# DoumanAsh/compu

Measured on AMD Instinct MI355X. Metric: decompressed GB/s (whole node), batched 64 KiB DEFLATE blocks; % HBM peak, higher is better.
Workload: dtype u8

## Files before the change

### compu_amd/csrc/inflate_unit.h

```cpp
#pragma once
#include "chip_internal.h"
#include "wave_checksums.h"

namespace chip {

typedef uint32_t u32x2 __attribute__((ext_vector_type(2)));
typedef uint32_t u32x4 __attribute__((ext_vector_type(4)));
typedef u32x4 u32x4_u __attribute__((aligned(1)));
typedef u32x4 u32x4_a4 __attribute__((aligned(4)));
template <typename T>
__device__ __forceinline__ GAS T *rdfirst_gptr(T *p)
{
    return (GAS T *)rdfirst_ptr(p);
}

#ifndef CHIP_PHASE_FN
#define CHIP_PHASE_FN __attribute__((always_inline))
#endif

#ifndef CHIP_INFLATE_SPEC
#define CHIP_INFLATE_SPEC 0
#endif
#ifndef CHIP_INFLATE_MARKERS
#define CHIP_INFLATE_MARKERS 0
// ... 471 lines not shown
    if (allow_gzip && b0 == 0x1f && b1 == 0x8b) {
        wrap = 2;
        if (avail < 4) return CHIP_NEED_INPUT;
        const uint32_t flg = gin[3];
        if (gin[2] != 8) return Z_DATA_ERROR;
        if (flg & 0xe0) return Z_DATA_ERROR;
        if (avail < 10) return CHIP_NEED_INPUT;
        uint32_t k = 10;
        if (flg & 4) {
            if (avail < k + 2) return CHIP_NEED_INPUT;
            uint32_t xlen = gin[k] | ((uint32_t)gin[k + 1] << 8);
            k += 2;
            if (avail - k < xlen) return CHIP_NEED_INPUT;
            k += xlen;
        }
        for (uint32_t bit = 8; bit <= 16; bit <<= 1) {
            if (!(flg & bit)) continue;
            for (;;) {
                uint32_t idx = k + lane_id();
                uint64_t z = __ballot(idx < avail && gin[idx] == 0);
                if (z) {
                    k += (uint32_t)__ffsll((long long)z);
                    break;
                }
                if (avail - k <= 64) return CHIP_NEED_INPUT;
                k += 64;
            }
        }
        if (flg & 2) {
            if (avail < k + 2) return CHIP_NEED_INPUT;
            uint32_t crc = wave_crc32(tab, gin, k);
            if ((crc & 0xffffu) != (gin[k] | ((uint32_t)gin[k + 1] << 8))) return Z_DATA_ERROR;
            k += 2;
        }
        hdr = k;
        return ST_RUNNING;
    }
    if (!allow_zlib) return Z_DATA_ERROR;
    if (((b0 << 8) | b1) % 31u) return Z_DATA_ERROR;
    if ((b0 & 15u) != 8) return Z_DATA_ERROR;
    if ((b0 >> 4) + 8 > 15) return Z_DATA_ERROR;
    wrap = 1;
    hdr = 2;
    if (b1 & 0x20) {
        if (avail < 6) return CHIP_NEED_INPUT;
        hdr = 6;
        return CHIP_NEED_DICT;
    }
    return ST_RUNNING;
}

struct __attribute__((packed)) U32u { uint32_t v; };
struct __attribute__((packed)) U16u { uint16_t v; };
struct __attribute__((packed)) U128u { uint32_t x, y, z, w; };
typedef LDS_AS uint8_t lds_u8;

__device__ void wave_copy_stored(uint8_t *gdst, const uint32_t *g32, uint32_t total_dw, uint32_t so, uint32_t n)
{
    const uint32_t lane = lane_id();
    const uint8_t *gsrc = (const uint8_t *)g32 + so;
    uint32_t head = (uint32_t)((16u - ((uintptr_t)gdst & 15u)) & 15u);
    if (head > n) head = n;
    if (lane < head) gdst[lane] = gsrc[lane];
    uint32_t done = head;
    const uint32_t body = (n - done) & ~15u;
    if (body) {
        uint4 *d16 = (uint4 *)(gdst + done);
        const U128u *s16 = (const U128u *)(gsrc + done);
        const uint32_t cnt = body >> 4;
        uint32_t i = lane;
#ifdef CHIP_STORED_NT_LD
#define CHIP_STORED_LD(p) __builtin_nontemporal_load(p)
#else
#define CHIP_STORED_LD(p) (*(p))
#endif
#ifndef CHIP_STORED_PLAIN_ST
#define CHIP_STORED_ST(v, p) __builtin_nontemporal_store(v, p)
#else
#define CHIP_STORED_ST(v, p) (*(p) = (v))
#endif
#ifndef CHIP_STORED_DEPTH
#define CHIP_STORED_DEPTH 2
#endif
        for (; i + 64u * (CHIP_STORED_DEPTH - 1) < cnt; i += 64u * CHIP_STORED_DEPTH) {
            u32x4 v[CHIP_STORED_DEPTH];
#pragma unroll
            for (int k = 0; k < CHIP_STORED_DEPTH; k++) v[k] = CHIP_STORED_LD((const u32x4_u *)(s16 + i + 64u * k));
#pragma unroll
            for (int k = 0; k < CHIP_STORED_DEPTH; k++) CHIP_STORED_ST(v[k], (u32x4 *)(d16 + i + 64u * k));
        }
        for (; i < cnt; i += 64u) {
            const U128u a = s16[i];
            d16[i] = make_uint4(a.x, a.y, a.z, a.w);
        }
        done += body;
    }
    const uint32_t tail = n - done;
    if (lane < tail) gdst[done + lane] = gsrc[done + lane];
    (void)total_dw;
}

__device__ __forceinline__ uint32_t small_mod(uint32_t off, uint32_t d)
{
    uint32_t q = (uint32_t)(((float)off + 0.5f) * __builtin_amdgcn_rcpf((float)d));
    return off - q * d;
}
struct ChunkLds {
    uint32_t *out;
    uint2 *mq;
    uint32_t *tok;
    lds_u8 *trash;
};

__device__ __forceinline__ ChunkLds chunk_lds(WaveLds &L)
{
    ChunkLds c;
    c.out = L.fl.out;
    c.mq = L.fl.mq;
    c.tok = L.fl.tok;
    c.trash = (lds_u8 *)L.fl.trash;
    return c;
}

__device__ __forceinline__ void lds_put(lds_u8 *d, lds_u8 *trash, const U128u &v, uint32_t n)
{
    ((LDS_AS U32u *)(n >= 4 ? d : trash))->v = v.x;
    ((LDS_AS U32u *)((n >= 8 ? d : trash) + 4))->v = v.y;
    ((LDS_AS U32u *)((n >= 12 ? d : trash) + 8))->v = v.z;
    ((LDS_AS U32u *)((n >= 16 ? d : trash) + 12))->v = v.w;
    const uint32_t w = n < 4 ? v.x : n < 8 ? v.y : n < 12 ? v.z : v.w;
    lds_u8 *const t = d + (n & 12u);
    const bool two = (n & 2u) != 0, one = (n & 1u) != 0;
    ((LDS_AS U16u *)(two ? t : trash))->v = (uint16_t)w;
    *(one ? (two ? t + 2 : t) : trash) = (uint8_t)(two ? w >> 16 : w);
}

__device__ __forceinline__ void copy_one_match(lds_u8 *img, const uint8_t *base, uint32_t mis, uint32_t x, uint32_t len, uint32_t dist)
{
    const uint32_t lane = lane_id();
    const int32_t sx = (int32_t)x - (int32_t)dist;
    for (uint32_t i = lane; i < len; i += 64) {
        const int32_t s = sx + (int32_t)(dist >= len ? i : small_mod(i, dist));
        uint8_t b = 0;
        if (s < (int32_t)mis) b = ((GAS const uint8_t *)base)[s];
        if (s >= (int32_t)mis) b = img[s];
        img[x + i] = b;
    }
    LSYNC();
}

struct Round {
    uint32_t x, len, dist;
    bool glob;
    U128u v0, v1;
};

__device__ __forceinline__ void round_issue(Round &r, const ChunkLds &C, const uint8_t *base, uint32_t mis, uint32_t qh, uint32_t nr,
                                            bool glob_ok)
{
    const uint32_t lane = lane_id();
    const bool act = lane < nr;
    const uint32_t qi = (qh + lane) & (MQ_CAP - 1u);
    const uint2 e = C.mq[qi];
    r.x = e.x;
    const uint32_t ld = act ? e.y : 0u;
    r.len = ld & 0xffffu;
    r.dist = ld >> 16;
    const int32_t sx = (int32_t)r.x - (int32_t)r.dist;
    r.glob = glob_ok && r.len != 0 && r.len <= COPY_LANE_MAX && sx + (int32_t)r.len <= (int32_t)mis;
    r.v0 = U128u{0, 0, 0, 0};
    r.v1 = U128u{0, 0, 0, 0};
#ifndef CHIP_EXP_NO_GLOB
    if (r.glob) {
        const u32x4_u t = *(GAS const u32x4_u *)(base + sx);
        r.v0 = U128u{t.x, t.y, t.z, t.w};
    }
#endif
#ifndef CHIP_EXP_NO_GLOB
    if (r.glob && r.len > 16u) {
        const u32x4_u t = *(GAS const u32x4_u *)(base + sx + 16);
        r.v1 = U128u{t.x, t.y, t.z, t.w};
    }
#endif
}

__device__ __forceinline__ void round_finish(const Round &r, const ChunkLds &C, const uint8_t *base, uint32_t mis STAT_PARAM)
{
    const uint32_t lane = lane_id();
    lds_u8 *const img = (lds_u8 *)C.out;
    const int32_t sx = (int32_t)r.x - (int32_t)r.dist;
    uint64_t pend = __ballot(r.len != 0);
    STAT_ADD(14, 1);
    while (pend) {
        const uint32_t f = (uint32_t)__ffsll((long long)pend) - 1u;
        const uint32_t wp = rdlane(r.x, f);
        const bool mine = (pend >> lane) & 1ull;
        const bool loc = sx >= (int32_t)mis && (uint32_t)sx + r.len <= wp;
        const bool ready = mine && r.len <= COPY_LANE_MAX && (r.glob || loc);
        const uint64_t rm = __ballot(ready);
        if (!((rm >> f) & 1ull)) {
            STAT_ADD(15, 1);
            copy_one_match(img, base, mis, wp, rdlane(r.len, f), rdlane(r.dist, f));
            pend &= pend - 1ull;
            continue;
        }
        STAT_ADD(12, 1);
        uint32_t rem = ready ? r.len : 0u;
#pragma unroll
        for (uint32_t it = 0; it < COPY_LANE_MAX / 16; it++) {
            if (it && !__any(rem != 0)) break;
            U128u v = it ? r.v1 : r.v0;
            if (rem && !r.glob) {
                const lds_u8 *sp = img + sx + (int32_t)(16u * it);
                v.x = ((const LDS_AS U32u *)sp)->v;
                v.y = ((const LDS_AS U32u *)(sp + 4))->v;
                v.z = ((const LDS_AS U32u *)(sp + 8))->v;
                v.w = ((const LDS_AS U32u *)(sp + 12))->v;
            }
            const uint32_t n = rem < 16u ? rem : 16u;
            lds_put(img + r.x + 16u * it, C.trash, v, n);
            rem -= n;
        }
        LSYNC();
        pend &= ~rm;
    }
}

__device__ __forceinline__ uint32_t lane_gather(uint32_t x, uint32_t src)
{
    return (uint32_t)__builtin_amdgcn_ds_bpermute((int)(src << 2), (int)x);
}

__device__ uint32_t token_end(const WaveLds &L, const InWin &w, uint32_t p, bool second)
{
    const uint32_t i = p >> 5;
    const uint32_t d0 = i < w.total_dw ? w.g32[i] : 0u, d1 = i + 1u < w.total_dw ? w.g32[i + 1u] : 0u, d2 = i + 2u < w.total_dw ? w.g32[i + 2u] : 0u;
    const uint32_t lo = __builtin_amdgcn_alignbit(d1, d0, p), hi = __builtin_amdgcn_alignbit(d2, d1, p);
    const uint32_t r = L.lit_root[lo & ((1u << LIT_ROOT) - 1u)];
    const uint32_t e = pool_at(L, r, lo);
    const uint32_t n1 = __builtin_amdgcn_ubfe(e, 10, 5);
    const uint32_t w2 = __builtin_amdgcn_alignbit(hi, lo, n1);
    if (!(e & F_LEN)) {
        if (!second) return p + n1;
        const uint32_t r2 = L.lit_root[w2 & ((1u << LIT_ROOT) - 1u)];
        return p + n1 + __builtin_amdgcn_ubfe(pool_at(L, r2, w2), 10, 5);
    }
    uint32_t m = L.dist_root[w2 & ((1u << DIST_ROOT) - 1u)];
    if (m & D_LONG) m = dist_sub_at(L, m, w2);
    return p + n1 + (m & 15u) + __builtin_amdgcn_ubfe(m, 4, 4);
}

__device__ __attribute__((always_inline)) uint32_t overflow_bit(const WaveLds &L, const InWin &w, const uint32_t *grow, uint32_t ntok, uint32_t npieces,
                                                           uint32_t cstart, uint32_t run0, uint32_t xcap, uint32_t B)
{
    const uint32_t lane = lane_id();
    const uint32_t pfirst = lane < npieces ? L.fl.pk[2u * lane] : 0xffffffffu;
    const uint32_t pdelta = lane < npieces ? L.fl.pk[2u * lane + 1u] : 0u;
    uint32_t run = run0;
    for (uint32_t g = cstart; g < ntok; g += 64u) {
        const uint32_t t = g + lane < ntok ? g + lane : ntok - 1u;
        uint32_t k = 0;
        for (uint32_t q = 0; q < npieces; q++) k += rdlane(pfirst, q) <= t ? 1u : 0u;
        const uint32_t d = lane_gather(pdelta, k - 1u);
        const uint32_t krow = (t + d) & 0xffffu, rb = d >> 16;
        const uint32_t tok = grow[rb + row_word(krow)];
        uint32_t olen = tok_olen(tok);
        if (g + lane >= ntok) olen = 0;
        const uint32_t incl = wave_incl_scan(olen);
        const uint64_t over = __ballot(olen != 0 && run + incl > xcap);
        if (over) {
            const uint32_t f = (uint32_t)__ffsll((long long)over) - 1u;
            const uint32_t rbf = rdlane(rb, f), kf = rdlane(krow, f);
            const uint32_t owner = ((rbf / (8u * ROW_TOKENS)) << 3) | ((rbf % (8u * ROW_TOKENS)) >> 2);
            const bool both = rdlane(run + incl - 1u, f) <= xcap;
            uint32_t p = B + owner * S_BITS;
            for (uint32_t j = 0; j <= kf; j++) {
                const uint32_t tj = rdfirst(grow[rbf + row_word(j)]);
                p = rdfirst(token_end(L, w, p, (tj >> 31) != 0 && (j < kf || both)));
            }
            return p;
        }
        run += rdlane(incl, 63u);
    }
    return 0;
}

__device__ CHIP_PHASE_FN bool flush_tokens(WaveLds &L, const uint32_t *grow_, uint32_t ntok_, uint32_t npieces_, uint8_t *gout_, uint32_t &opos_,
                             uint32_t cap_, int32_t &status, uint32_t (&ovf)[3] STAT_PARAM)
{
    const uint32_t lane = lane_id();
    const uint32_t *const grow = rdfirst_ptr(grow_);
    uint8_t *const gout = rdfirst_ptr(gout_);
    const uint32_t ntok = rdfirst(ntok_), npieces = rdfirst(npieces_), cap = rdfirst(cap_);
    uint32_t opos = rdfirst(opos_);
    const ChunkLds C = chunk_lds(L);
    lds_u8 *const img = (lds_u8 *)C.out;
    if (ntok == 0) return true;
    const uint32_t pfirst = lane < npieces ? L.fl.pk[2u * lane] : 0xffffffffu;
    const uint32_t pdelta = lane < npieces ? L.fl.pk[2u * lane + 1u] : 0u;
    uint32_t before = 0;
    uint32_t nfirst = 0;
    uint32_t dcur = 0;
    uint32_t gnext = 0;
    uint32_t slot_w = 0;
    const uint32_t tok_lds = rdfirst((uint32_t)(uintptr_t)(LDS_AS uint32_t *)C.tok);
    auto fetch = [&]() {
        const uint32_t g = gnext;
        uint32_t d = dcur;
        while (nfirst - g < 64u) {
            dcur = rdlane(pdelta, before);
            d = lane >= nfirst - g ? dcur : d;
            before++;
            const uint32_t nx = rdlane(pfirst, before & 63u);
            nfirst = before < npieces ? nx : 0xffffffffu;
        }
        const uint32_t t = min(g + lane, ntok - 1u);
        gnext = g + 64u;
        const uint32_t krow = (t + d) & 0xffffu;
        const uint32_t *src = grow + ((d >> 16) + row_word(krow));
        const uint32_t dst = tok_lds + 256u * slot_w;
        uint32_t keep;
        asm volatile("s_mov_b32 %0, m0\n\ts_mov_b32 m0, %2\n\ts_nop 0\n\tglobal_load_lds_dword %1, off\n\ts_mov_b32 m0, %0"
                     : "=&s"(keep)
                     : "v"(src), "s"(dst)
                     : "memory");
        slot_w = (slot_w + 1u) & (TOK_RING - 1u);
    };
    WSYNC();
    uint32_t c0 = 0;
    uint32_t slot_r = 0;
#pragma unroll
    for (uint32_t k = 0; k < TOK_RING; k++) fetch();
    bool fresh = true;
    uint32_t mis = 0, run = 0, nq = 0, qh = 0, prod0 = 0, cstart = 0;
    uint8_t *base = gout;
    bool glob_ok = false, inflight = false;
    Round R;
    for (;;) {
        if (fresh) {
            STAT_ADD(13, 1);
            mis = (uint32_t)((uintptr_t)(gout + opos) & 3u);
            base = gout + opos - mis;
            glob_ok = cap - opos >= 16u;
            run = mis;
            prod0 = opos - mis;
            nq = qh = 0;
            cstart = c0;
            fresh = false;
        }
        static_assert(TOK_RING == 4, "the wait below counts three younger ring loads");
        asm volatile("s_waitcnt vmcnt(3)" ::: "memory");
        const uint32_t t = C.tok[64u * slot_r + lane];
        const bool ismatch = (t & 512u) != 0;
        const uint32_t len = ismatch ? t & 0x1ffu : 0u;
        const uint32_t val = ismatch ? __builtin_amdgcn_ubfe(t, 10, 16) + 1u : t;
        const uint32_t left = ntok - c0;
        const bool pair = (int32_t)t < 0;
        uint32_t olen = ismatch ? len : 1u + (t >> 31);
        olen = lane < left ? olen : 0u;
        const uint32_t incl = wave_incl_scan(olen);
        const uint32_t start = run + incl - olen;
        const uint32_t total = rdlane(incl, 63u);
        const uint64_t lenm = __ballot(len != 0);
        uint32_t nacc;
        bool ending, too_far = false;
        if (left >= 64u && run + total <= CHUNK_BYTES && (opos >= 32768u || (__ballot(val > prod0 + start) & lenm) == 0)) {
            asm volatile("; the common group" ::: "memory");
            const uint32_t qi = __builtin_amdgcn_mbcnt_hi((uint32_t)(lenm >> 32), __builtin_amdgcn_mbcnt_lo((uint32_t)lenm, nq)) & (MQ_CAP - 1u);
            *(len == 0 ? img + start : C.trash) = (uint8_t)val;
            *(pair ? img + start + 1u : C.trash) = (uint8_t)(t >> 16);
            *(len != 0 ? &C.mq[qi] : (uint2 *)(uint8_t *)C.trash) = make_uint2(start, len | (val << 16));
            nq += (uint32_t)__popcll(lenm);
            c0 += 64u;
            run += total;
            nacc = 64u;
            ending = c0 >= ntok;
        } else {
            const uint32_t nvalid = left < 64u ? left : 64u;
            const uint64_t validm = nvalid == 64u ? ~0ull : (1ull << nvalid) - 1ull;
            const uint64_t nofit = __ballot(incl > CHUNK_BYTES - run) & validm;
            const uint64_t badm = __ballot(val > prod0 + start) & lenm & validm;
            const uint64_t stopm = nofit | badm;
            nacc = stopm ? (uint32_t)__ffsll((long long)stopm) - 1u : nvalid;
            too_far = stopm != 0 && ((badm & ~nofit) >> nacc) & 1ull;
            if (stopm && !too_far && run != mis) nacc = 0;
            if (lane < nacc && len == 0) img[start] = (uint8_t)val;
            if (lane < nacc && pair) img[start + 1u] = (uint8_t)(t >> 16);
            const uint64_t mm = lenm & (nacc == 64u ? ~0ull : (1ull << nacc) - 1ull);
            if (lane < nacc && len != 0) {
                const uint32_t qi = __builtin_amdgcn_mbcnt_hi((uint32_t)(mm >> 32), __builtin_amdgcn_mbcnt_lo((uint32_t)mm, nq)) & (MQ_CAP - 1u);
                C.mq[qi] = make_uint2(start, len | (val << 16));
            }
            nq += (uint32_t)__popcll(mm);
            c0 += nacc;
            if (stopm) {
                if (nacc) run = rdlane(start, nacc);
            } else {
                run += total;
            }
            ending = stopm != 0 || c0 >= ntok;
        }
        LSYNC();
        STAT_ACC(16);
        if (nq - qh >= 64u || ending) {
            do {
                if (inflight) {
                    round_finish(R, C, base, mis STAT_ARG);
                    inflight = false;
                }
                const uint32_t pq = nq - qh;
                if (pq >= 64u || (ending && pq != 0)) {
                    const uint32_t nr = pq < 64u ? pq : 64u;
                    round_issue(R, C, base, mis, qh, nr, glob_ok);
                    qh += nr;
                    inflight = true;
                }
            } while (ending && inflight);
        }
        STAT_ACC(17);
        if (nacc == 64u) {
            fetch();
            slot_r = (slot_r + 1u) & (TOK_RING - 1u);
        } else if (nacc != 0 && c0 < ntok) {
            gnext = c0;
            before = (uint32_t)__popcll(__ballot(pfirst < c0));
            dcur = rdlane(pdelta, before - 1u);
            {
                const uint32_t nx = rdlane(pfirst, before & 63u);
                nfirst = before < npieces ? nx : 0xffffffffu;
            }
            asm volatile("s_waitcnt vmcnt(0)" ::: "memory");
            slot_r = slot_w = 0;
#pragma unroll
            for (uint32_t k = 0; k < TOK_RING; k++) fetch();
        }
        if (!ending) continue;
        const uint32_t xcap = cap - (opos - mis);
        {
            const uint32_t xe = run < xcap ? run : xcap;
            for (uint32_t xq = 16u + 16u * lane; xq + 16u <= xe; xq += 1024u) *(GAS u32x4_a4 *)(base + xq) = *(const LDS_AS u32x4 *)(img + xq);
            const uint32_t xt = xe < 16u ? 16u : xe & ~15u;
            const uint32_t xb = lane < 16u ? lane : xt + (lane - 16u);
            if (lane < 32u && xb >= mis && xb < xe) ((GAS uint8_t *)base)[xb] = img[xb];
        }
        WSYNC();
        STAT_ACC(18);
        opos += run - mis;
        opos_ = opos;
        const bool no_room = opos > cap || (too_far && opos == cap);
        if (no_room || too_far) {
            if (no_room) {
                opos_ = cap;
                ovf[0] = cstart;
                ovf[1] = mis;
                ovf[2] = xcap;
            }
            status = no_room ? CHIP_NEED_OUTPUT : Z_DATA_ERROR;
            return false;
        }
        if (c0 >= ntok) return true;
        fresh = true;
    }
}
constexpr size_t SCRATCH_WORDS = ROWS_WORDS;


enum : uint32_t { R_JOIN = 1, R_LIMIT = 2, R_EOB = 3, R_NEED_INPUT = 4, R_BAD = 5 };

__device__ CHIP_PHASE_FN uint32_t walk_round(WaveLds &L, const InWin &w, const uint32_t B_, const uint32_t end_bit_, uint32_t *rows_, const uint32_t xt_bits,
                                             uint32_t &ntok_out, uint32_t &term_why, uint32_t &term_pos STAT_PARAM)
{
    const uint32_t lane = lane_id();
    const uint32_t B = rdfirst(B_), end_bit = rdfirst(end_bit_);
    GAS const uint32_t *const g32 = rdfirst_gptr(w.g32);
    const uint32_t total_dw = rdfirst(w.total_dw);
    GAS uint32_t *const myrow = rdfirst_gptr(rows_) + row_base(lane);
    const uint32_t D0 = B >> 5;
    WSYNC();
    {
        constexpr uint32_t WIN_Q = WIN_DW / 4, WIN_R = WIN_DW % 4;
        constexpr uint32_t BM_A = (WIN_DW + 3u) & ~3u;
        constexpr uint32_t BM_Q = (2u * WIN_DW - BM_A) / 4, BM_TAIL = (2u * WIN_DW - BM_A) % 4;
        constexpr uint32_t EDGE_LO = WIN_R + (BM_A - WIN_DW);
        constexpr uint32_t EDGE_LANES = 4u + EDGE_LO + BM_TAIL;
        constexpr uint32_t PER_LANE = (WIN_Q + 63) / 64;
        static_assert(offsetof(WaveLds, w.win) == 0 && offsetof(WaveLds, w.bm) == 4 * WIN_DW && BM_Q <= WIN_Q && EDGE_LANES <= 64, "window staging");
        uint32_t *const ww = L.w.win;
        const uint32_t rem = total_dw - D0;
        static_assert(PER_LANE <= 4, "the quads per lane below");
        auto quad = [&](uint32_t j) -> u32x4 {
            const uint32_t k = 64u * j + lane;
            if ((64u * j + 63u < WIN_Q || k < WIN_Q) && 4u * k + 4u <= rem) return *(GAS const u32x4_a4 *)(g32 + D0 + 4u * k);
            return u32x4{0, 0, 0, 0};
        };
        const u32x4 v0 = quad(0), v1 = quad(1), v2 = quad(2), v3 = quad(3);
        uint32_t ni = 4u * (rem >> 2) + lane;
        bool nput = ni < rem && ni < 4u * WIN_Q;
        if (lane >= 4u) {
            const uint32_t j = lane - 4u;
            ni = j < EDGE_LO ? 4u * WIN_Q + j : 2u * WIN_DW - BM_TAIL + (j - EDGE_LO);
            nput = j < EDGE_LO + BM_TAIL;
        }
        uint32_t nv = 0;
        if (nput && ni < rem && ni < WIN_DW) nv = g32[D0 + ni];
#pragma unroll
        for (uint32_t j = 0; j < PER_LANE; j++) {
            const uint32_t k = 64u * j + lane;
            if (64u * j + 63u < WIN_Q || k < WIN_Q) *(u32x4 *)(ww + 4u * k) = j == 0 ? v0 : j == 1 ? v1 : j == 2 ? v2 : v3;
            if (64u * j + 63u < BM_Q || k < BM_Q) *(u32x4 *)(ww + BM_A + 4u * k) = u32x4{0, 0, 0, 0};
        }
        if (nput) ww[ni] = nv;
    }
    LSYNC();
    STAT_ACC(1);
    STAT_ADD(8, 1);
    const uint32_t s0 = B + lane * S_BITS;
    const uint32_t own_end = s0 + S_BITS;
    uint32_t hard = own_end + xt_bits;
    {
        const uint32_t sr_end = B + 64u * S_BITS;
        hard = hard < sr_end ? hard : sr_end;
        hard = hard < end_bit ? hard : end_bit;
    }
    const uint32_t wbase = 32u * D0;
    const uint32_t own_end_r = own_end - wbase, hard_r = hard - wbase;
    uint32_t q = s0 - wbase, tl = 0, nst = 0;
    uint32_t jb = 0, z = 0;
    bool run = s0 < end_bit;
    uint32_t nx;
    {
        const uint32_t *wp = (const uint32_t *)((const uint8_t *)L.w.win + ((q >> 3) & ~3u));
        nx = __builtin_amdgcn_alignbit(wp[1], wp[0], q);
    }
    auto token = [&](uint32_t &tok) -> bool {
        const uint32_t p = q;
        const uint32_t a = (p >> 3) & ~3u;
        const uint32_t bit = 1u << (p & 31u);
        const uint32_t mine = p < own_end_r ? bit : 0u;
        const uint32_t old = atomicOr((uint32_t *)((uint8_t *)L.w.bm + a), mine);
        jb = old & bit & ~mine;
        const uint32_t *wp = (const uint32_t *)((const uint8_t *)L.w.win + a);
        const uint32_t d0 = wp[0], d1 = wp[1], d2 = wp[2];
        const uint32_t lo = __builtin_amdgcn_alignbit(d1, d0, p), hi = __builtin_amdgcn_alignbit(d2, d1, p);
        const uint32_t r = L.lit_root[nx & ((1u << LIT_ROOT) - 1u)];
        const uint32_t e = pool_at(L, r, nx);
        const uint32_t n1 = __builtin_amdgcn_ubfe(e, 10, 5);
        const uint32_t msk = (uint32_t)((int32_t)e >> 31);
        const uint32_t w2 = __builtin_amdgcn_alignbit(hi, lo, n1);
        uint32_t m = L.dist_root[w2 & ((1u << DIST_ROOT) - 1u)] & msk;
#ifndef CHIP_EXP_NO_PAIR
        const uint32_t p2 = p + n1;
        const uint32_t r2 = L.lit_root[w2 & ((1u << LIT_ROOT) - 1u)];
        const uint32_t mw2 = *(const uint32_t *)((const uint8_t *)L.w.bm + ((p2 >> 3) & ~3u));
#endif
        if (__any((m & D_LONG) != 0)) {
            asm volatile("; long distance codes");
            if (m & D_LONG) m = dist_sub_at(L, m, w2);
        }
#ifndef CHIP_EXP_NO_PAIR
        const uint32_t e2 = pool_at(L, r2, w2);
        const uint32_t mk2 = __builtin_amdgcn_ubfe(mw2, p2, 1);
#endif
        const uint32_t cl2 = m & 15u, eb2 = __builtin_amdgcn_ubfe(m, 4, 4);
        const uint32_t dm1 = ((m >> 8) << eb2) + __builtin_amdgcn_ubfe(w2, cl2, eb2);
        z = (e & (F_HALT | F_INV)) | (m & D_BAD);
        tl = n1 + cl2 + eb2;
#ifndef CHIP_EXP_NO_PAIR
        const uint32_t n2 = __builtin_amdgcn_ubfe(e2, 10, 5);
        const bool pair = ((e | e2) & (F_LEN | F_HALT)) == 0 && p2 + n2 <= hard_r && mk2 == 0;
        tl += pair ? n2 : 0u;
        const uint32_t pr = pair ? (e2 & 0x00ff0000u) | 0x80000000u : 0u;
#else
        const uint32_t pr = 0;
#endif
        static_assert((15 + 5) + (15 + 13) == 48 && 64 - 48 >= LIT_ROOT + (15 - LIT_ROOT), "the next step's index bits are in hi:lo");
        nx = (uint32_t)((((uint64_t)hi << 32) | lo) >> (tl & 63u));
        q = p + tl;
        if ((jb | z) != 0 || q > hard_r) return false;
        const uint32_t v = __builtin_amdgcn_ubfe(lo, e, e >> 5) + __builtin_amdgcn_ubfe(e, 16, 10);
        tok = (dm1 << 10) | v | pr;
        return true;
    };
    bool full = false;
    while (__any(run)) {
        STAT_ADD(11, 1);
        uint32_t t4[4];
#pragma unroll
        for (int k = 0; k < 4; k++) asm volatile("" : "=v"(t4[k]));
        uint32_t took = 0;
        if (run) {
            if (nst + 4u > ROW_TOKENS) {
                run = false;
                full = true;
            } else {
                bool ok = token(t4[0]);
                if (ok) {
                    took = 1;
                    ok = token(t4[1]);
                    if (ok) {
                        took = 2;
                        ok = token(t4[2]);
                        if (ok) {
                            took = 3;
                            ok = token(t4[3]);
                            if (ok) took = 4;
                        }
                    }
                }
                run = ok;
            }
        }
        if (took) *(GAS u32x4 *)(myrow + 8u * nst) = u32x4{t4[0], t4[1], t4[2], t4[3]};
        nst += took;
    }
    const bool dropped = s0 < end_bit && !full;
    const uint32_t pn = q + wbase;
    const uint32_t p = pn - (dropped ? tl : 0u);
    uint32_t why = R_LIMIT;
    if (s0 < end_bit && !full) {
        if (jb) why = R_JOIN;
        else if (pn > end_bit) why = R_NEED_INPUT;
        else if (z) why = z == F_HALT ? (uint32_t)R_EOB : (uint32_t)R_BAD;
    }
    STAT_ADD(21, __popcll(__ballot(nst != 0)));
    STAT_ACC(2);
    const uint32_t rel = p - B;
    const uint32_t jl = why == R_JOIN ? (__umul24(rel, SEG_MAGIC) >> SEG_SHIFT) & 63u : lane;
    uint32_t a_join = 0;
    if (__any(why == R_JOIN)) {
        const uint32_t sj = B + jl * S_BITS;
        const uint32_t w0 = (sj >> 5) - D0;
        const uint32_t lo_cut = sj & 31u;
        const uint32_t nb = p - (sj & ~31u);
#pragma unroll
        for (uint32_t t = 0; t < SEG_WORDS; t++) {
            uint32_t mw = L.w.bm[w0 + t];
            if (t == 0) mw &= ~0u << lo_cut;
            const int32_t k = (int32_t)nb - 32 * (int32_t)t;
            const uint32_t keep = k <= 0 ? 0u : k >= 32 ? 0xffffffffu : (1u << k) - 1u;
            a_join += __popc(mw & keep);
        }
        if (why != R_JOIN) a_join = 0;
    }
    uint32_t node = 0;
    {
        uint32_t pw = jl;
#pragma unroll
        for (int r = 0; r < 6; r++) {
            const uint32_t nx = lane_gather(pw, node);
            if ((lane >> r) & 1u) node = nx;
            pw = lane_gather(pw, pw);
        }
    }
    const uint32_t prev = wave_shr1(node);
    const bool fresh = lane == 0 || node != prev;
    const uint32_t e_nst = lane_gather(nst, node);
    const uint32_t g_a0 = lane_gather(a_join, prev);
    const uint32_t e_a0 = lane == 0 ? 0u : g_a0;
    const uint32_t cnt = (fresh && e_nst > e_a0) ? e_nst - e_a0 : 0u;
    const uint32_t incl = wave_incl_scan(cnt);
    const uint64_t nonempty = __ballot(cnt != 0);
    WSYNC();
    if (cnt) {
        const uint32_t k = (uint32_t)__popcll(nonempty & lanemask_lt()), first = incl - cnt;
        L.fl.pk[2u * k] = first;
        L.fl.pk[2u * k + 1u] = ((e_a0 - first) & 0xffffu) | (row_base(node) << 16);
    }
    const uint32_t kz = rdlane(node, 63);
    term_why = rdlane(why, kz);
    term_pos = rdlane(p, kz);
    ntok_out = rdlane(incl, 63u);
    WSYNC();
    STAT_ACC(3);
    STAT_ADD(9, __popcll(nonempty));
    STAT_ADD(10, ntok_out);
    return (uint32_t)__popcll(nonempty);
}

__device__ CHIP_PHASE_FN bool count_tokens(WaveLds &L, const uint32_t *grow_, uint32_t ntok_, uint32_t npieces_, uint64_t &osize, int32_t &status SPEC_PARAM)
{
    const uint32_t lane = lane_id();
    GAS const uint32_t *const grow = rdfirst_gptr(grow_);
    const uint32_t ntok = rdfirst(ntok_), npieces = rdfirst(npieces_);
    if (ntok == 0) return true;
    const bool have = lane < npieces;
    const uint32_t pfirst = have ? L.fl.pk[2u * lane] : ntok;
    const uint32_t pdelta = have ? L.fl.pk[2u * lane + 1u] : 0u;
    const uint32_t pnext = lane + 1u < npieces ? L.fl.pk[2u * lane + 2u] : ntok;
    const uint32_t k0 = (pfirst + pdelta) & 0xffffu;
    const uint32_t kend = k0 + (have ? pnext - pfirst : 0u);
    GAS const uint32_t *const row = grow + (pdelta >> 16);
    uint32_t sum = 0;
    for (uint32_t kq = k0 & ~3u; __any(kq < kend); kq += 4u) {
        if (kq < kend) {
            const u32x4 t = *(GAS const u32x4 *)(row + 8u * kq);
            const uint32_t t4[4] = {t.x, t.y, t.z, t.w};
#pragma unroll
            for (uint32_t j = 0; j < 4; j++)
                if (kq + j >= k0 && kq + j < kend) sum += tok_olen(t4[j]);
        }
    }
    const uint32_t incl = wave_incl_scan(sum);
    const uint32_t olo = rdfirst((uint32_t)osize), ohi = rdfirst((uint32_t)(osize >> 32));
#if CHIP_INFLATE_SPEC
    if (ohi == 0 && olo < 32768u) {
        uint32_t at = olo + incl - sum, reach = 0;
        for (uint32_t kq = k0 & ~3u; __any(kq < kend); kq += 4u) {
            if (kq < kend) {
                const u32x4 t = *(GAS const u32x4 *)(row + 8u * kq);
                const uint32_t t4[4] = {t.x, t.y, t.z, t.w};
#pragma unroll
                for (uint32_t j = 0; j < 4; j++)
                    if (kq + j >= k0 && kq + j < kend) {
                        const uint32_t dist = __builtin_amdgcn_ubfe(t4[j], 10, 16) + 1u;
                        if ((t4[j] & 512u) != 0 && dist > at && dist - at > reach) reach = dist - at;
                        at += tok_olen(t4[j]);
                    }
            }
        }
        const uint32_t far = rdlane(wave_incl_max_scan(reach), 63u);
        if (far > sp_reach) sp_reach = far;
    }
    (void)status;
#else
    if (ohi == 0 && olo < 32768u) {
        uint32_t at = olo + incl - sum, badat = 0xffffffffu;
        for (uint32_t kq = k0 & ~3u; __any(kq < kend); kq += 4u) {
            if (kq < kend) {
                const u32x4 t = *(GAS const u32x4 *)(row + 8u * kq);
                const uint32_t t4[4] = {t.x, t.y, t.z, t.w};
#pragma unroll
                for (uint32_t j = 0; j < 4; j++)
                    if (kq + j >= k0 && kq + j < kend) {
                        const bool ismatch = (t4[j] & 512u) != 0;
                        if (ismatch && __builtin_amdgcn_ubfe(t4[j], 10, 16) + 1u > at && badat == 0xffffffffu) badat = at;
                        at += tok_olen(t4[j]);
                    }
            }
        }
        const uint64_t badm = __ballot(badat != 0xffffffffu);
        if (badm) {
            osize = rdlane(badat, (uint32_t)__ffsll((long long)badm) - 1u);
            status = Z_DATA_ERROR;
            return false;
        }
    }
#endif
    osize = (((uint64_t)ohi << 32) | olo) + rdlane(incl, 63u);
    return true;
}

#if CHIP_INFLATE_MARKERS
#define MSYNC() __builtin_amdgcn_fence(__ATOMIC_SEQ_CST, "workgroup")
constexpr uint32_t MARK = 0x8000u, MARK_WINDOW = 32768u;
constexpr uint32_t LANE_COPY16 = 32;

__device__ __forceinline__ void copy_match16(GAS uint16_t *gout, uint32_t x, uint32_t len, uint32_t dist)
{
    const uint32_t lane = lane_id();
    const int32_t sx = (int32_t)x - (int32_t)dist;
    for (uint32_t i = lane; i < len; i += 64) {
        const int32_t s = sx + (int32_t)(dist >= len ? i : small_mod(i, dist));
        const uint16_t v = s < 0 ? (uint16_t)(MARK | (uint32_t)(s + (int32_t)MARK_WINDOW)) : gout[s];
        gout[x + i] = v;
// ... 611 lines not shown
```

Baseline: 356.8.

## Split token flush into specialized steady loop with hoisted distance test

Restructures flush_tokens so each chunk runs a tight inner steady loop specialized at compile time on whether the back-reference distance test is needed (opos < 32 KiB), with the slow tail handling moved out of the hot loop. The ring write slot is passed explicitly instead of kept as loop state, per-chunk state becomes loop-local constants, and the round's glob flag is carried as a ballot mask. Asm barriers pin the Round registers so their live ranges stay bounded. The aim is fewer branches and less register pressure in the common group path, at the cost of duplicated code and more complex control flow.

```diff
diff --git a/compu_amd/csrc/inflate_unit.h b/compu_amd/csrc/inflate_unit.h
--- a/compu_amd/csrc/inflate_unit.h
+++ b/compu_amd/csrc/inflate_unit.h
@@ -797,9 +797,8 @@
     uint32_t nfirst = 0;
     uint32_t dcur = 0;
     uint32_t gnext = 0;
-    uint32_t slot_w = 0;
     const uint32_t tok_lds = rdfirst((uint32_t)(uintptr_t)(LDS_AS uint32_t *)C.tok);
-    auto fetch = [&]() {
+    auto fetch = [&](const uint32_t slot_w) {
         const uint32_t g = gnext;
         uint32_t d = dcur;
         while (nfirst - g < 64u) {
@@ -819,102 +818,129 @@
                      : "=&s"(keep)
                      : "v"(src), "s"(dst)
                      : "memory");
-        slot_w = (slot_w + 1u) & (TOK_RING - 1u);
     };
     WSYNC();
     uint32_t c0 = 0;
     uint32_t slot_r = 0;
 #pragma unroll
-    for (uint32_t k = 0; k < TOK_RING; k++) fetch();
-    bool fresh = true;
-    uint32_t mis = 0, run = 0, nq = 0, qh = 0, prod0 = 0, cstart = 0;
-    uint8_t *base = gout;
-    bool glob_ok = false, inflight = false;
-    Round R;
+    for (uint32_t k = 0; k < TOK_RING; k++) fetch(k);
     for (;;) {
-        if (fresh) {
-            STAT_ADD(13, 1);
-            mis = (uint32_t)((uintptr_t)(gout + opos) & 3u);
-            base = gout + opos - mis;
-            glob_ok = cap - opos >= 16u;
-            run = mis;
-            prod0 = opos - mis;
-            nq = qh = 0;
-            cstart = c0;
-            fresh = false;
-        }
-        static_assert(TOK_RING == 4, "the wait below counts three younger ring loads");
-        asm volatile("s_waitcnt vmcnt(3)" ::: "memory");
-        const uint32_t t = C.tok[64u * slot_r + lane];
-        const bool ismatch = (t & 512u) != 0;
-        const uint32_t len = ismatch ? t & 0x1ffu : 0u;
-        const uint32_t val = ismatch ? __builtin_amdgcn_ubfe(t, 10, 16) + 1u : t;
-        const uint32_t left = ntok - c0;
-        const bool pair = (int32_t)t < 0;
-        uint32_t olen = ismatch ? len : 1u + (t >> 31);
-        olen = lane < left ? olen : 0u;
-        const uint32_t incl = wave_incl_scan(olen);
-        const uint32_t start = run + incl - olen;
-        const uint32_t total = rdlane(incl, 63u);
-        const uint64_t lenm = __ballot(len != 0);
-        uint32_t nacc;
-        bool ending, too_far = false;
-        if (left >= 64u && run + total <= CHUNK_BYTES && (opos >= 32768u || (__ballot(val > prod0 + start) & lenm) == 0)) {
-            asm volatile("; the common group" ::: "memory");
-            const uint32_t qi = __builtin_amdgcn_mbcnt_hi((uint32_t)(lenm >> 32), __builtin_amdgcn_mbcnt_lo((uint32_t)lenm, nq)) & (MQ_CAP - 1u);
-            *(len == 0 ? img + start : C.trash) = (uint8_t)val;
-            *(pair ? img + start + 1u : C.trash) = (uint8_t)(t >> 16);
-            *(len != 0 ? &C.mq[qi] : (uint2 *)(uint8_t *)C.trash) = make_uint2(start, len | (val << 16));
-            nq += (uint32_t)__popcll(lenm);
-            c0 += 64u;
+        STAT_ADD(13, 1);
+        const uint32_t mis = (uint32_t)((uintptr_t)(gout + opos) & 3u);
+        uint8_t *const base = gout + opos - mis;
+        const bool glob_ok = cap - opos >= 16u;
+        const uint32_t prod0 = opos - mis;
+        const uint32_t cstart = c0;
+        uint32_t run = mis, nq = 0, qh = 0;
+        Round R;
+        bool inflight = false;
+        uint64_t globm = 0;
+        uint32_t t, len, val, left, incl, start, total;
+        bool pair;
+        uint64_t lenm;
+        auto group = [&]() __attribute__((always_inline)) {
+            static_assert(TOK_RING == 4, "the wait below counts three younger ring loads");
+            asm volatile("s_waitcnt vmcnt(3)" ::: "memory");
+            t = C.tok[64u * slot_r + lane];
+            const bool ismatch = (t & 512u) != 0;
+            len = ismatch ? t & 0x1ffu : 0u;
+            val = ismatch ? __builtin_amdgcn_ubfe(t, 10, 16) + 1u : t;
+            left = ntok - c0;
+            pair = (int32_t)t < 0;
+            uint32_t olen = ismatch ? len : 1u + (t >> 31);
+            olen = lane < left ? olen : 0u;
+            incl = wave_incl_scan(olen);
+            start = run + incl - olen;
+            total = rdlane(incl, 63u);
+            lenm = __ballot(len != 0);
+        };
+        auto steady = [&](const bool dist_test) __attribute__((always_inline)) {
+            {
+                uint32_t u[11];
+#pragma unroll
+                for (int k = 0; k < 11; k++) asm volatile("" : "=v"(u[k]));
+                R.x = u[0], R.len = u[1], R.dist = u[2], R.glob = false;
+                R.v0 = U128u{u[3], u[4], u[5], u[6]};
+                R.v1 = U128u{u[7], u[8], u[9], u[10]};
+            }
+            for (;;) {
+                group();
+                if (left < 64u || run + total > CHUNK_BYTES) break;
+                if (dist_test && (__ballot(val > prod0 + start) & lenm) != 0) break;
+                if (dist_test)
+                    asm volatile("; a steady group, distances tested" ::: "memory");
+                else
+                    asm volatile("; a steady group" ::: "memory");
+                const uint32_t qi = __builtin_amdgcn_mbcnt_hi((uint32_t)(lenm >> 32), __builtin_amdgcn_mbcnt_lo((uint32_t)lenm, nq)) & (MQ_CAP - 1u);
+                *(len == 0 ? img + start : C.trash) = (uint8_t)val;
+                *(pair ? img + start + 1u : C.trash) = (uint8_t)(t >> 16);
+                *(len != 0 ? &C.mq[qi] : (uint2 *)(uint8_t *)C.trash) = make_uint2(start, len | (val << 16));
+                nq += (uint32_t)__popcll(lenm);
+                c0 += 64u;
+                run += total;
+                LSYNC();
+                STAT_ACC(16);
+                if (nq - qh >= 64u) {
+                    if (inflight) {
+                        R.glob = __builtin_amdgcn_inverse_ballot_w64(globm);
+                        round_finish(R, C, base, mis STAT_ARG);
+                    }
+                    round_issue(R, C, base, mis, qh, 64u, glob_ok);
+                    globm = __ballot(R.glob);
+                    qh += 64u;
+                    inflight = true;
+                }
+                STAT_ACC(17);
+                fetch(slot_r);
+                slot_r = (slot_r + 1u) & (TOK_RING - 1u);
+            }
+        };
+        if (opos < 32768u)
+            steady(true);
+        else
+            steady(false);
+        const uint32_t nvalid = left < 64u ? left : 64u;
+        const uint64_t validm = nvalid == 64u ? ~0ull : (1ull << nvalid) - 1ull;
+        const uint64_t nofit = __ballot(incl > CHUNK_BYTES - run) & validm;
+        const uint64_t badm = __ballot(val > prod0 + start) & lenm & validm;
+        const uint64_t stopm = nofit | badm;
+        uint32_t nacc = stopm ? (uint32_t)__ffsll((long long)stopm) - 1u : nvalid;
+        const bool too_far = stopm != 0 && ((badm & ~nofit) >> nacc) & 1ull;
+        if (stopm && !too_far && run != mis) nacc = 0;
+        if (lane < nacc && len == 0) img[start] = (uint8_t)val;
+        if (lane < nacc && pair) img[start + 1u] = (uint8_t)(t >> 16);
+        const uint64_t mm = lenm & (nacc == 64u ? ~0ull : (1ull << nacc) - 1ull);
+        if (lane < nacc && len != 0) {
+            const uint32_t qi = __builtin_amdgcn_mbcnt_hi((uint32_t)(mm >> 32), __builtin_amdgcn_mbcnt_lo((uint32_t)mm, nq)) & (MQ_CAP - 1u);
+            C.mq[qi] = make_uint2(start, len | (val << 16));
+        }
+        nq += (uint32_t)__popcll(mm);
+        c0 += nacc;
+        if (stopm) {
+            if (nacc) run = rdlane(start, nacc);
+        } else {
             run += total;
-            nacc = 64u;
-            ending = c0 >= ntok;
-        } else {
-            const uint32_t nvalid = left < 64u ? left : 64u;
-            const uint64_t validm = nvalid == 64u ? ~0ull : (1ull << nvalid) - 1ull;
-            const uint64_t nofit = __ballot(incl > CHUNK_BYTES - run) & validm;
-            const uint64_t badm = __ballot(val > prod0 + start) & lenm & validm;
-            const uint64_t stopm = nofit | badm;
-            nacc = stopm ? (uint32_t)__ffsll((long long)stopm) - 1u : nvalid;
-            too_far = stopm != 0 && ((badm & ~nofit) >> nacc) & 1ull;
-            if (stopm && !too_far && run != mis) nacc = 0;
-            if (lane < nacc && len == 0) img[start] = (uint8_t)val;
-            if (lane < nacc && pair) img[start + 1u] = (uint8_t)(t >> 16);
-            const uint64_t mm = lenm & (nacc == 64u ? ~0ull : (1ull << nacc) - 1ull);
-            if (lane < nacc && len != 0) {
-                const uint32_t qi = __builtin_amdgcn_mbcnt_hi((uint32_t)(mm >> 32), __builtin_amdgcn_mbcnt_lo((uint32_t)mm, nq)) & (MQ_CAP - 1u);
-                C.mq[qi] = make_uint2(start, len | (val << 16));
-            }
-            nq += (uint32_t)__popcll(mm);
-            c0 += nacc;
-            if (stopm) {
-                if (nacc) run = rdlane(start, nacc);
-            } else {
-                run += total;
-            }
-            ending = stopm != 0 || c0 >= ntok;
         }
         LSYNC();
         STAT_ACC(16);
-        if (nq - qh >= 64u || ending) {
-            do {
-                if (inflight) {
-                    round_finish(R, C, base, mis STAT_ARG);
-                    inflight = false;
-                }
-                const uint32_t pq = nq - qh;
-                if (pq >= 64u || (ending && pq != 0)) {
-                    const uint32_t nr = pq < 64u ? pq : 64u;
-                    round_issue(R, C, base, mis, qh, nr, glob_ok);
-                    qh += nr;
-                    inflight = true;
-                }
-            } while (ending && inflight);
-        }
+        for (;;) {
+            if (inflight) {
+                R.glob = __builtin_amdgcn_inverse_ballot_w64(globm);
+                round_finish(R, C, base, mis STAT_ARG);
+                inflight = false;
+            }
+            const uint32_t pq = nq - qh;
+            if (pq == 0) break;
+            const uint32_t nr = pq < 64u ? pq : 64u;
+            round_issue(R, C, base, mis, qh, nr, glob_ok);
+            globm = __ballot(R.glob);
+            qh += nr;
+            inflight = true;
+        }
+        asm volatile("" ::"v"(R.v0.x), "v"(R.v0.y), "v"(R.v0.z), "v"(R.v0.w), "v"(R.v1.x), "v"(R.v1.y), "v"(R.v1.z), "v"(R.v1.w));
         STAT_ACC(17);
         if (nacc == 64u) {
-            fetch();
+            fetch(slot_r);
             slot_r = (slot_r + 1u) & (TOK_RING - 1u);
         } else if (nacc != 0 && c0 < ntok) {
             gnext = c0;
@@ -925,11 +951,10 @@
                 nfirst = before < npieces ? nx : 0xffffffffu;
             }
             asm volatile("s_waitcnt vmcnt(0)" ::: "memory");
-            slot_r = slot_w = 0;
-#pragma unroll
-            for (uint32_t k = 0; k < TOK_RING; k++) fetch();
-        }
-        if (!ending) continue;
+            slot_r = 0;
+#pragma unroll
+            for (uint32_t k = 0; k < TOK_RING; k++) fetch(k);
+        }
         const uint32_t xcap = cap - (opos - mis);
         {
             const uint32_t xe = run < xcap ? run : xcap;
@@ -954,7 +979,6 @@
             return false;
         }
         if (c0 >= ntok) return true;
-        fresh = true;
     }
 }
 constexpr size_t SCRATCH_WORDS = ROWS_WORDS;
```

Result: faster. 376.3, median of 6 (+5.5%).
